# luo-yining/CFDBench

Hardware: AMD Instinct MI355X
Metric: train frames/sec (64x64x2), Auto-FNO cavity (higher is better)
Workload: dtype f32; 1 GPU; BASELINE configs[1]: Auto-FNO train step (fwd+nMSE+bwd+Adam), Fno2d(L=4,hidden=20,modes=12,p=5), 64x64, batch 256/GPU, fp32, random-init weights; act_pieces=3, global_batch=256, parallelism=dp1, graph=False, settle_steps=30

## Files before the change

cfdbench_amd/csrc/cfd_common.h:

```cpp
#pragma once
#include <cfd_intrinsics.h>
#include <hip/hip_runtime.h>

#include "../../include/cfdbench_amd.h"

void cfd_set_error(const char* fmt, ...);

enum { CFD_TUNE_MIX_NWV = 0, CFD_TUNE_WGRAD_WG, CFD_TUNE_FUSED_VARIANT, CFD_TUNE_BLOCK_FUSE, CFD_TUNE_GENERAL_B3, CFD_TUNE_HEAD_BLOCKS, CFD_TUNE_EXACT_FP32, CFD_TUNE_CONV6_GRID, CFD_TUNE_CONV6_WGRAD_MUL, CFD_TUNE_CONVT_MFMA, CFD_TUNE_CONV1_MFMA, CFD_TUNE_SIDE_STREAM, CFD_TUNE_ACT_PIECES, CFD_TUNE_BLOCK_GEN,
    CFD_TUNE_GEMM_TILE, CFD_TUNE_GEMM_SPLITS, CFD_TUNE_BLOCK_WIDE, CFD_TUNE_HEAD_WAVES, CFD_TUNE_STEM_FUSE, CFD_TUNE_MODE_MFMA, CFD_TUNE_MODE_BC, CFD_TUNE_STEM_DFT, CFD_TUNE_GEMM_B3, CFD_TUNE_COUNT };
int cfd_tune_get(int which);

#define CFD_REQUIRE(cond, code, ...)      \
    do {                                  \
        if (!(cond)) {                    \
            cfd_set_error(__VA_ARGS__);   \
            return (code);                \
        }                                 \
    } while (0)

#define CFD_REQUIRE_ALIGNED(ptr, bytes, fn, name) \
    CFD_REQUIRE(((size_t)(ptr) & (size_t)((bytes) - 1)) == 0, CFD_ERR_UNSUPPORTED, "%s: %s must be %d-byte aligned", fn, name, (int)(bytes))

#define CFD_LAUNCH_CHECK(name)                                                        \
    do {                                                                              \
        hipError_t e_ = hipGetLastError();                                            \
        if (e_ != hipSuccess) {                                                       \
            cfd_set_error("%s: HIP launch failed: %s", name, hipGetErrorString(e_));  \
            return CFD_ERR_HIP;                                                       \
        }                                                                             \
    } while (0)

#define CFD_TRY(expr)              \
    do {                           \
        int rc_ = (expr);          \
        if (rc_ != CFD_OK) return rc_; \
    } while (0)

hipStream_t cfd_side_fork(hipStream_t main, int use);
int cfd_side_join(hipStream_t main, hipStream_t side);
bool cfd_prof_active();

struct CfdProfScope {
    hipStream_t st;
    int idx;
    CfdProfScope(const char* name, hipStream_t s, double bytes = 0.0, double flops = 0.0);
    ~CfdProfScope();
};
#define CFD_PROF_CAT2(a, b) a##b
#define CFD_PROF_CAT(a, b) CFD_PROF_CAT2(a, b)
#define CFD_PROF(name, st) CfdProfScope CFD_PROF_CAT(cfd_prof_scope_, __LINE__)(name, st)
#define CFD_PROF_W(name, st, bytes, flops) \
    CfdProfScope CFD_PROF_CAT(cfd_prof_scope_, __LINE__)(name, st, (double)(bytes), (double)(flops))

#define CFD_KB_TMAX 5
struct cfd_plan {
    int H, W, m1, m2;
    int NJ;
    int KX;
    int T;
    int SA;
    int SB;
    int n_fwd, n_inv;
    float* d_fwd;
    float* d_inv;
    void* d_fwd_b3;
    void* d_inv_b3;
    int E;
    float* d_tail;
    void* d_fwd_g;
    void* d_inv_g;
    int NJG, NHG, n_fwd_gv, n_inv_gv;
    float* d_clhw;
    float* d_gx;
    float* d_gy;
    int many;
    float* d_many_fwd;
    float* d_many_inv;
};

struct CfdManyDims {
    int Hk, Hp, Wk, Wq, N1p, K2, R2p, R4;
};
__host__ __device__ static inline CfdManyDims cfd_many_dims(int H, int W, int m1, int m2) {
    CfdManyDims d;
    d.Hk = (H + 3) / 4 * 4;
    d.Hp = (H + 15) / 16 * 16;
    d.Wk = (W + 3) / 4 * 4;
    d.Wq = (W + 15) / 16 * 16;
    d.N1p = (2 * m2 + 15) / 16 * 16;
    d.K2 = (2 * m2 + 3) / 4 * 4;
    d.R2p = (2 * m1 + 15) / 16 * 16;
    d.R4 = (2 * m1 + 3) / 4 * 4;
    return d;
}
int cfd_int_dft_many(const cfd_plan* p, const float* x, float* xh, int nimg, int act_in, void* stream);
int cfd_int_idft_many(const cfd_plan* p, const float* z, const float* addend, const float* aprev, float* out, int nimg, int epi, void* stream);

static inline size_t cfd_align_up(size_t v, size_t a) { return (v + a - 1) / a * a; }

#define CFD_DT_F32 0
#define CFD_DT_BF16 1
template <typename TA>
__device__ __forceinline__ float cfd_ld(const TA* p) { return (float)*p; }
template <typename TA>
__device__ __forceinline__ void cfd_st(TA* p, float v) { *p = (TA)v; }
static inline size_t cfd_dt_size(int dt) { return dt == CFD_DT_BF16 ? 2 : 4; }
__device__ __forceinline__ float4 cfd_ld4(const float* p) { return *reinterpret_cast<const float4*>(p); }
__device__ __forceinline__ float4 cfd_ld4(const __bf16* p) {
    typedef __bf16 bf16x4_ __attribute__((ext_vector_type(4)));
    const bf16x4_ t = *reinterpret_cast<const bf16x4_*>(p);
    return make_float4((float)t[0], (float)t[1], (float)t[2], (float)t[3]);
}

struct __attribute__((packed, aligned(4))) cfd_f4u { float x, y, z, w; };
__device__ __forceinline__ float4 cfd_ld4u(const float* p) {
    const cfd_f4u v = *reinterpret_cast<const cfd_f4u*>(p);
    return make_float4(v.x, v.y, v.z, v.w);
}
__device__ __forceinline__ void cfd_st4u(float* p, float4 v) { *reinterpret_cast<cfd_f4u*>(p) = cfd_f4u{v.x, v.y, v.z, v.w}; }

int cfd_int_spectral_dft(const cfd_plan* p, const void* x, float* xh, int nimg, int act_in, int dt, void* stream);
bool cfd_int_dft_stem_ok(const cfd_plan* p, int B, int in_chan, int P, int C, const void* inputs, const void* mask, const void* a0);
int cfd_int_spectral_dft_stem(const cfd_plan* p, const float* inputs, const float* mask, const float* cp, const float* w, const float* bias,
                              float* a0, float* xh, int B, int P, int C, void* stream);
int cfd_int_spectral_idft(const cfd_plan* p, const float* z, const void* addend, const void* aprev, void* out, int nimg, int epi,
                          int dt, void* stream);
int cfd_int_spectral_idft_grad(const cfd_plan* p, const float* z, const float* addend, const void* aprev, float* out, int nimg,
                               int dt, void* stream);
int cfd_int_chanmix(const void* in, const float* w, const float* bias, void* out, int B, int Ci, int Co, int HW, int act_in,
                    int transpose, int dt, void* stream);
int cfd_int_fno_stem_fwd(const cfd_plan* p, const float* inputs, const float* mask, const float* case_params, const float* w,
                         const float* bias, void* out, int B, int in_chan, int P, int C, int dt, void* stream);
int cfd_int_fno_head_fwd(const void* a, const float* mask, const float* label, const float* w1, const float* b1, const float* w2,
                         const float* b2, float* preds, float* sums, void* ws, int B, int C, int Hd, int Co, int HW, int act_in,
                         int dt, void* stream);

#define CFD_PAD_COORD_GY 128
#define CFD_PAD_COORD_FLOATS 256
int cfd_int_stem_pad(const float* inputs, const float* mask, const float* case_params, const float* w, const float* bias, float* out,
                     float* coords, int B, int in_chan, int P, int C, int H, int W, int pad, void* stream);
int cfd_int_pad_crop(const float* in, float* out, long n, int H, int W, int pad, void* stream);
int cfd_int_pad_embed(const float* in, float* out, long n, int H, int W, int pad, void* stream);

int cfd_int_fno_ingrad(const float* g0, const float* w, float* d_inputs, float* d_case_params, void* ws, size_t ws_bytes, int B, int in_chan,
                       int P, int C, int HW, void* stream);

#define CFD_WIDE_MAX 128
int cfd_int_wide_mix(const cfd_plan* p, const float* xh, const float* w1, const float* w2, float* z, int B, int Cin, int Cout,
                     int conj_t, void* stream);
int cfd_int_wide_wgrad(const cfd_plan* p, const float* xh, const float* gh, float* gw1, float* gw2, int B, int Cin, int Cout,
                       void* stream);
int cfd_int_wide_chanmix(const float* in, const float* w, const float* bias, float* out, int B, int Ci, int Co, int HW, int act_in,
                         int transpose, void* stream, const float* dgelu = nullptr);
size_t cfd_int_wide_chan_wgrad_workspace_bytes(int B, int Ci, int Co, int HW);
int cfd_int_wide_chan_wgrad(const float* g, const float* in, float* gw, float* gb, void* ws, int B, int Ci, int Co, int HW, int act_in,
                            void* stream);
int cfd_int_wide_stem_bwd(const cfd_plan* p, const float* g, const float* inputs, const float* mask, const float* case_params, float* gw,
                          float* gb, void* ws, int B, int in_chan, int P, int C, void* stream);
int cfd_int_wide_head_bwd(const float* a, const float* mask, const float* label, const float* preds, const float* gext, const float* coef,
                          const float* w1, const float* b1, const float* w2, float* ga, float* gw1, float* gb1, float* gw2, float* gb2,
                          void* ws, int B, int C, int Co, int HW, int act_in, void* stream);
int cfd_int_wide_stem_fwd(const cfd_plan* p, const float* inputs, const float* mask, const float* case_params, const float* w,
// ... 298 lines not shown
```

cfdbench_amd/csrc/pointwise.hip:

```cpp
#include "cfd_common.h"
#include "cfd_tail.h"

template <int CP, typename TA>
__global__ __launch_bounds__(256) void k_stem_fwd(const float* __restrict__ inputs, const float* __restrict__ mask,
                                                  const float* __restrict__ cp, const float* __restrict__ gx,
                                                  const float* __restrict__ gy, const float* __restrict__ w,
                                                  const float* __restrict__ bias, TA* __restrict__ out, int B,
                                                  int in_chan, int P, int C, int H, int W) {
    __shared__ float s_w[32 * CP];
    __shared__ float s_b[CP];
    const int F = in_chan + 3 + P;
    {
        constexpr int NV = (32 * CP + 255) / 256;
        float wv[NV];
#pragma unroll
        for (int k = 0; k < NV; ++k) {
            const int i = threadIdx.x + 256 * k, f = i / CP, o = i % CP;
            wv[k] = w[(o < C ? o : C - 1) * F + (f < F ? f : F - 1)];
        }
        float bv = bias[(int)threadIdx.x < C ? threadIdx.x : C - 1];
#pragma unroll
        for (int k = 0; k < NV; ++k) {
            const int i = threadIdx.x + 256 * k, f = i / CP, o = i % CP;
            wv[k] = cfd_opaque_f(wv[k]);
// ... 443 lines not shown
    const size_t ea = sizeof(TA);
    const int vec = (HW % 4 == 0 && ((uintptr_t)in % (4 * ea)) == 0 && ((uintptr_t)out % 16) == 0)   ? 4
                    : (HW % 2 == 0 && ((uintptr_t)in % (2 * ea)) == 0 && ((uintptr_t)out % 8) == 0) ? 2
                                                                                                    : 1;
    CFD_PROF_W(transpose ? "k_chanmix_t" : (act ? "k_chanmix_act" : "k_chanmix"), st, B * HW * ((double)ea * Ci + 4.0 * Co),
               2.0 * B * HW * (double)Ci * Co);
    const bool ap3 = sizeof(TA) == 4 && cfd_act_pieces() == 3;
#define CFD_CB3_P(M_, V_, A_, P_) \
    hipLaunchKernelGGL((k_chanmix_b3<M_, V_, A_, TA, P_>), dim3(blocks), dim3(256), 0, st, in, w, bias, out, B, Ci, Co, HW, transpose)
#define CFD_CB3(M_, V_, A_)                                                                   \
    do {                                                                                      \
        if constexpr (sizeof(TA) == 4) { if (ap3) CFD_CB3_P(M_, V_, A_, 3); else CFD_CB3_P(M_, V_, A_, 2); } \
        else CFD_CB3_P(M_, V_, A_, 2);                                                        \
    } while (0)
#define CFD_CB3_V(M_)                                                      \
    do {                                                                   \
        if (vec == 4) { if (act) CFD_CB3(M_, 4, true); else CFD_CB3(M_, 4, false); } \
        else if (vec == 2) { if (act) CFD_CB3(M_, 2, true); else CFD_CB3(M_, 2, false); } \
        else { if (act) CFD_CB3(M_, 1, true); else CFD_CB3(M_, 1, false); }  \
    } while (0)
    if (Co <= 16) CFD_CB3_V(1);
    else CFD_CB3_V(2);
#undef CFD_CB3_V
#undef CFD_CB3
#undef CFD_CB3_P
    CFD_LAUNCH_CHECK("cfd_chanmix");
    return CFD_OK;
}

template <int CPO, int VEC>
static int launch_chanmix(const float* in, const float* w, const float* bias, float* out, int B, int Ci, int Co, int HW,
                          int act, int transpose, hipStream_t st) {
    const long total = (long)B * (HW / VEC);
    int blocks = (int)((total + 255) / 256);
    if (blocks > 4096) blocks = 4096;
    CFD_PROF_W(transpose ? "k_chanmix_t" : (act ? "k_chanmix_act" : "k_chanmix"), st, 4.0 * B * HW * ((double)Ci + Co),
               2.0 * B * HW * (double)Ci * Co);
    if (act)
        hipLaunchKernelGGL((k_chanmix<CPO, VEC, true>), dim3(blocks), dim3(256), 0, st, in, w, bias, out, B, Ci, Co, HW, transpose);
    else
        hipLaunchKernelGGL((k_chanmix<CPO, VEC, false>), dim3(blocks), dim3(256), 0, st, in, w, bias, out, B, Ci, Co, HW, transpose);
    CFD_LAUNCH_CHECK("cfd_chanmix");
    return CFD_OK;
}

int cfd_int_chanmix(const void* in, const float* w, const float* bias, void* out, int B, int Ci, int Co, int HW, int act_in,
                    int transpose, int dt, void* stream) {
    if (dt == CFD_DT_F32) return cfd_chanmix((const float*)in, w, bias, (float*)out, B, Ci, Co, HW, act_in, transpose, stream);
    CFD_REQUIRE(in && w && out && B >= 0 && Ci >= 1 && Co >= 1 && HW >= 1 && Ci <= 32 && Co <= 32, CFD_ERR_INVALID_ARG, "cfd_chanmix: bad arguments");
    if (B == 0) return CFD_OK;
    hipStream_t st = (hipStream_t)stream;
    if (cfd_tune_get(CFD_TUNE_EXACT_FP32) != 1)
        return launch_chanmix_b3<__bf16>((const __bf16*)in, w, bias, (float*)out, B, Ci, Co, HW, act_in, transpose, st);
    const int VEC = HW % 2 == 0 ? 2 : 1;
    const long total = (long)B * (HW / VEC);
    int blocks = (int)((total + 255) / 256);
    if (blocks > 4096) blocks = 4096;
    CFD_PROF_W(act_in ? "k_chanmix_act" : "k_chanmix", st, B * HW * (2.0 * Ci + 4.0 * Co), 2.0 * B * HW * (double)Ci * Co);
#define CFD_CMB(CPV, VW, A_)                                                                                                  \
    hipLaunchKernelGGL((k_chanmix<CPV, VW, A_, __bf16, float>), dim3(blocks), dim3(256), 0, st, (const __bf16*)in, w, bias, (float*)out, B, \
                       Ci, Co, HW, transpose)
#define CFD_CMB_VA(CPV)                                                    \
    do {                                                                   \
        if (VEC == 2) { if (act_in) CFD_CMB(CPV, 2, true); else CFD_CMB(CPV, 2, false); } \
        else { if (act_in) CFD_CMB(CPV, 1, true); else CFD_CMB(CPV, 1, false); }          \
    } while (0)
    if (Co <= 8) CFD_CMB_VA(8);
    else if (Co <= 16) CFD_CMB_VA(16);
    else if (Co <= 24) CFD_CMB_VA(24);
    else CFD_CMB_VA(32);
#undef CFD_CMB_VA
#undef CFD_CMB
    CFD_LAUNCH_CHECK("cfd_chanmix(bf16 storage)");
    return CFD_OK;
}

extern "C" int cfd_chanmix(const float* in, const float* w, const float* bias, float* out, int B, int Ci, int Co, int HW,
                           int act_in, int transpose, void* stream) {
    CFD_REQUIRE(in && w && out, CFD_ERR_INVALID_ARG, "cfd_chanmix: NULL pointer");
    CFD_REQUIRE(B >= 0 && Ci >= 1 && Co >= 1 && HW >= 1, CFD_ERR_INVALID_ARG, "cfd_chanmix: bad sizes");
    CFD_REQUIRE(Ci <= CFD_WIDE_MAX && Co <= CFD_WIDE_MAX, CFD_ERR_UNSUPPORTED, "cfd_chanmix: Ci=%d Co=%d (max %d) unsupported", Ci, Co,
                CFD_WIDE_MAX);
    if (B == 0) return CFD_OK;
    if (Ci > 32 || Co > 32) return cfd_int_wide_chanmix(in, w, bias, out, B, Ci, Co, HW, act_in, transpose, stream);
    hipStream_t st = (hipStream_t)stream;
    if (cfd_tune_get(CFD_TUNE_EXACT_FP32) != 1)
        return launch_chanmix_b3<float>(in, w, bias, out, B, Ci, Co, HW, act_in, transpose, st);
    const bool v4 = HW % 4 == 0 && ((uintptr_t)in % 16) == 0 && ((uintptr_t)out % 16) == 0;
    const bool v2 = HW % 2 == 0 && ((uintptr_t)in % 8) == 0 && ((uintptr_t)out % 8) == 0;
#define CFD_CM(CPV, VW)                                                                               \
    return (VW == 4 && v4) ? launch_chanmix<CPV, VW>(in, w, bias, out, B, Ci, Co, HW, act_in, transpose, st) \
           : v2            ? launch_chanmix<CPV, 2>(in, w, bias, out, B, Ci, Co, HW, act_in, transpose, st)  \
                           : launch_chanmix<CPV, 1>(in, w, bias, out, B, Ci, Co, HW, act_in, transpose, st)
    if (Co <= 8) CFD_CM(8, 4);
    if (Co <= 16) CFD_CM(16, 4);
    if (Co <= 24) CFD_CM(24, 2);
    CFD_CM(32, 2);
#undef CFD_CM
}

struct StemSrc {
    const float* mask;
    const float* cp;
    const float* gx;
    const float* gy;
    int in_chan, P, W;
};

template <int VEC>
__device__ __forceinline__ void cfd_ld8px(const float* __restrict__ src, int px, int hw, bool ok, float (&v)[8]) {
#pragma unroll
    for (int j = 0; j < 8; ++j) v[j] = 0.f;
    if (!ok) return;
    if constexpr (VEC == 4) {
#pragma unroll
        for (int k = 0; k < 2; ++k)
            if (px + 4 * k < hw) {
                const float4 t = *reinterpret_cast<const float4*>(src + 4 * k);
                v[4 * k] = t.x; v[4 * k + 1] = t.y; v[4 * k + 2] = t.z; v[4 * k + 3] = t.w;
            }
    } else {
#pragma unroll
        for (int k = 0; k < 2; ++k) {
            if (px + 4 * k + 3 < hw) {
                const float4 t = cfd_ld4u(src + 4 * k);
                v[4 * k] = t.x; v[4 * k + 1] = t.y; v[4 * k + 2] = t.z; v[4 * k + 3] = t.w;
            } else {
#pragma unroll
                for (int j = 0; j < 4; ++j)
                    if (px + 4 * k + j < hw) v[4 * k + j] = src[4 * k + j];
            }
        }
    }
}

template <int VEC>
__device__ __forceinline__ void cfd_ld8px(const __bf16* __restrict__ src, int px, int hw, bool ok, float (&v)[8]) {
#pragma unroll
    for (int j = 0; j < 8; ++j) v[j] = 0.f;
    if (!ok) return;
    if constexpr (VEC == 4) {
        if (px + 4 < hw) {
            const bf16x8 t = *reinterpret_cast<const bf16x8*>(src);
#pragma unroll
            for (int j = 0; j < 8; ++j) v[j] = (float)t[j];
        } else if (px < hw) {
#pragma unroll
            for (int j = 0; j < 4; ++j) v[j] = (float)src[j];
        }
    } else {
#pragma unroll
        for (int j = 0; j < 8; ++j)
            if (px + j < hw) v[j] = (float)src[j];
    }
}

template <int MT, int NT, int VEC, bool ACT, bool STEM, typename TIN, int AP>
__global__ __launch_bounds__(256) void k_chan_wgrad(const float* __restrict__ g, const TIN* __restrict__ in,
                                                    StemSrc ss, float* __restrict__ part, int B, int Ci, int Co,
                                                    int HW) {
    __shared__ float s_red[4 * MT * NT * 4 * 64];
    const int lane = threadIdx.x & 63, wave = threadIdx.x >> 6;
    const int q = lane >> 4, n = lane & 15;
    const f32x4 zero = {0.f, 0.f, 0.f, 0.f};
    f32x4 acc[MT][NT];
#pragma unroll
    for (int a = 0; a < MT; ++a)
#pragma unroll
        for (int c = 0; c < NT; ++c) acc[a][c] = zero;
    const int cpb = (HW + 31) / 32;
    const int total = B * cpb;
    const int CiIn = STEM ? ss.in_chan : Ci;
    auto load = [&](int ch, float (&av)[MT][8], float (&bv)[NT][8]) {
        const int b = (int)((unsigned)ch / (unsigned)cpb);
        const int px = (ch - b * cpb) * 32 + 8 * q;
#pragma unroll
        for (int a = 0; a < MT; ++a) {
            const int o = 16 * a + n;
            const float* src = g + ((size_t)b * Co + (o < Co ? o : 0)) * HW + px;
            cfd_ld8px<VEC>(src, px, HW, o < Co, av[a]);
        }
#pragma unroll
        for (int c = 0; c < NT; ++c) {
            const int i = 16 * c + n;
            if (i < CiIn) {
                const TIN* src = in + ((size_t)b * CiIn + i) * HW + px;
                cfd_ld8px<VEC>(src, px, HW, true, bv[c]);
            } else {
                const int f = STEM ? i - ss.in_chan : -1;
                const int row0 = STEM ? px / ss.W : 0, col0 = STEM ? px - row0 * ss.W : 0;
                const bool same_row = STEM && (ss.W % 8 == 0);
                if constexpr (STEM && VEC == 4) {
                    if (same_row && (((uintptr_t)ss.mask | (uintptr_t)ss.gy) % 16) == 0) {
                        const float* p8 = nullptr;
                        const float* p1 = nullptr;
                        float s = 0.f;
                        if (i == Ci) s = 1.f;
                        else if (f == 0) { if (ss.mask) p8 = ss.mask + (size_t)b * HW + px; else s = 1.f; }
                        else if (f == 1) p1 = ss.gx + row0;
                        else if (f == 2) p8 = ss.gy + col0;
                        else if (f < 3 + ss.P) p1 = ss.cp + (size_t)b * ss.P + (f - 3);
                        float4 t0 = make_float4(0.f, 0.f, 0.f, 0.f), t1 = t0;
                        if (p8) {
                            if (px < HW) t0 = *reinterpret_cast<const float4*>(p8);
                            if (px + 4 < HW) t1 = *reinterpret_cast<const float4*>(p8 + 4);
                        } else {
                            if (p1) s = *p1;
                            if (px < HW) t0 = make_float4(s, s, s, s);
                            if (px + 4 < HW) t1 = make_float4(s, s, s, s);
                        }
                        bv[c][0] = t0.x; bv[c][1] = t0.y; bv[c][2] = t0.z; bv[c][3] = t0.w;
                        bv[c][4] = t1.x; bv[c][5] = t1.y; bv[c][6] = t1.z; bv[c][7] = t1.w;
                        continue;
                    }
                }
                float cval = 0.f;
                const float* plane = nullptr;
                const float* tab = nullptr;
                bool by_row = false;
                if (i == Ci) cval = 1.f;
                else if constexpr (STEM) {
                    if (f == 0) { if (ss.mask) plane = ss.mask + (size_t)b * HW + px; else cval = 1.f; }
                    else if (f == 1) { tab = ss.gx; by_row = true; }
                    else if (f == 2) tab = ss.gy;
                    else if (f < 3 + ss.P) cval = ss.cp[(size_t)b * ss.P + (f - 3)];
                }
                if (plane) {
                    if (((uintptr_t)ss.mask % (4 * VEC)) == 0) cfd_ld8px<VEC>(plane, px, HW, true, bv[c]);
                    else cfd_ld8px<1>(plane, px, HW, true, bv[c]);
                } else if (tab) {
                    int row = row0, col = col0;
#pragma unroll
                    for (int j = 0; j < 8; ++j) {
                        bv[c][j] = (px + j < HW) ? tab[by_row ? row : col] : 0.f;
                        if (++col >= ss.W) { col = 0; ++row; }
                    }
                } else {
#pragma unroll
                    for (int j = 0; j < 8; ++j) bv[c][j] = (px + j < HW) ? cval : 0.f;
                }
            }
        }
    };
    const int stride = (int)gridDim.x * 4;
    int ch = (int)blockIdx.x * 4 + wave;
    float av[MT][8], bv[NT][8], avn[MT][8], bvn[NT][8];
    if (ch < total) load(ch, av, bv);
    while (ch < total) {
        const int nx = ch + stride;
        if (nx < total) load(nx, avn, bvn);
        cfd_sched_fence();
        if constexpr (ACT) {
#pragma unroll
            for (int c = 0; c < NT; ++c)
                if (16 * c + n < CiIn) {
#pragma unroll
                    for (int j = 0; j < 8; j += 2) { const cfd_f2 g2 = cfd_gelu2(cfd_f2{bv[c][j], bv[c][j + 1]}); bv[c][j] = g2.x; bv[c][j + 1] = g2.y; }
                }
        }
        {
            CfdAct8<AP> as[MT], bs[NT];
#pragma unroll
            for (int a = 0; a < MT; ++a) as[a] = cfd_act_split8<AP>(av[a]);
#pragma unroll
            for (int c = 0; c < NT; ++c) bs[c] = cfd_act_split8<AP>(bv[c]);
#pragma unroll
            for (int k = 0; k < cfd_nterm_aa(AP); ++k)
#pragma unroll
                for (int a = 0; a < MT; ++a)
#pragma unroll
                    for (int c = 0; c < NT; ++c)
                        acc[a][c] = cfd_mfma16x16x32_bf16(as[a].p[cfd_term_aa_a(AP, k)], bs[c].p[cfd_term_aa_b(AP, k)], acc[a][c]);
        }
        cfd_sched_fence();
#pragma unroll
        for (int a = 0; a < MT; ++a)
#pragma unroll
            for (int j = 0; j < 8; ++j) av[a][j] = avn[a][j];
#pragma unroll
        for (int c = 0; c < NT; ++c)
#pragma unroll
            for (int j = 0; j < 8; ++j) bv[c][j] = bvn[c][j];
        ch = nx;
    }
#pragma unroll
    for (int a = 0; a < MT; ++a)
#pragma unroll
        for (int c = 0; c < NT; ++c)
#pragma unroll
            for (int r = 0; r < 4; ++r) s_red[((wave * MT * NT + a * NT + c) * 4 + r) * 64 + lane] = acc[a][c][r];
    __syncthreads();
    const int NW = Ci + 1;
    float* dst = part + (size_t)blockIdx.x * Co * NW;
    const size_t nb = 1;
    for (int e = threadIdx.x; e < MT * NT * 4 * 64; e += blockDim.x) {
        const int ln = e & 63, r = (e >> 6) & 3, tile = e >> 8;
        const int a = tile / NT, c = tile % NT;
        const int o = 16 * a + 4 * (ln >> 4) + r, i = 16 * c + (ln & 15);
        if (o < Co && i < NW) {
            float s = 0.f;
#pragma unroll
            for (int wv = 0; wv < 4; ++wv) s += s_red[((wv * MT * NT + tile) * 4 + r) * 64 + ln];
            dst[(size_t)(o * NW + i) * nb] = s;
        }
    }
}

__global__ __launch_bounds__(256) void k_wgrad_reduce(const float* __restrict__ part, int nblk, float* __restrict__ gw,
                                                      float* __restrict__ gb, int Co, int Ci) {
    __shared__ float s_scr[64];
    chan_wgrad_reduce_group(blockIdx.x, part, nblk, gw, gb, Co, Ci, s_scr);
}

static int wgrad_blocks(int B, int HW) {
    const long chunks = (long)B * ((HW + 31) / 32);
    long blocks = (chunks + 7) / 8;
    if (blocks > 1024) blocks = 1024;
    const long fill = (chunks + 3) / 4 < 256 ? (chunks + 3) / 4 : 256;
    if (blocks < fill) blocks = fill;
    if (blocks < 1) blocks = 1;
    return (int)blocks;
}

extern "C" size_t cfd_chan_wgrad_workspace_bytes(int B, int Ci, int Co, int HW) {
    if (B <= 0) return 0;
    if (Ci > 32 || Co > 32) return cfd_int_wide_chan_wgrad_workspace_bytes(B, Ci, Co, HW);
    return (size_t)wgrad_blocks(B, HW) * Co * (Ci + 1) * sizeof(float);
}

template <bool STEM, typename TIN = float>
static int launch_wgrad(const float* g, const TIN* in, StemSrc ss, float* gw, float* gb, void* ws, int B, int Ci,
                        int Co, int HW, int act, hipStream_t st, ChanWgradTail* defer = nullptr) {
    const int blocks = wgrad_blocks(B, HW);
    CFD_REQUIRE((long)B * ((HW + 31) / 32) < (1L << 30), CFD_ERR_UNSUPPORTED, "cfd_chan_wgrad: B * ceil(HW / 32) = %ld chunks (max 2^30)",
                (long)B * ((HW + 31) / 32));
    const int MT = (Co + 15) / 16, NT = (Ci + 1 + 15) / 16;
    const int vec = sizeof(TIN) == 2 ? ((HW % 8 == 0 && ((uintptr_t)g % 16) == 0 && ((uintptr_t)in % 16) == 0) ? 4 : 1)
                    : (HW % 4 == 0 && ((uintptr_t)g % 16) == 0 && ((uintptr_t)in % 16) == 0)  ? 4
                    : (HW % 2 == 0 && ((uintptr_t)g % 8) == 0 && ((uintptr_t)in % 8) == 0) ? 2
                                                                                            : 1;
    float* part = (float*)ws;
    const bool ap3 = sizeof(TIN) == 4 && cfd_act_pieces() == 3;
#define CFD_WG_P(M_, N_, V_, A_, P_)                                                                             \
    hipLaunchKernelGGL((k_chan_wgrad<M_, N_, V_, A_, STEM, TIN, P_>), dim3(blocks), dim3(256), 0, st, g, in, ss, part, B, \
                       Ci, Co, HW)
#define CFD_WG(M_, N_, V_, A_)                                                                \
    do {                                                                                      \
        if constexpr (sizeof(TIN) == 4) { if (ap3) CFD_WG_P(M_, N_, V_, A_, 3); else CFD_WG_P(M_, N_, V_, A_, 2); } \
        else CFD_WG_P(M_, N_, V_, A_, 2);                                                     \
    } while (0)
#define CFD_WG_VA(M_, N_)                                                                     \
    do {                                                                                      \
        if (vec == 4) { if (act) CFD_WG(M_, N_, 4, true); else CFD_WG(M_, N_, 4, false); }    \
        else if (vec == 2) { if constexpr (sizeof(TIN) == 4) { if (act) CFD_WG(M_, N_, 2, true); else CFD_WG(M_, N_, 2, false); } } \
        else { if (act) CFD_WG(M_, N_, 1, true); else CFD_WG(M_, N_, 1, false); }             \
    } while (0)
    {
    CFD_PROF_W(STEM ? "k_chan_wgrad_stem" : "k_chan_wgrad", st, (double)B * HW * (4.0 * Co + sizeof(TIN) * (STEM ? 3 : Ci)),
               2.0 * B * HW * (double)Co * (Ci + 1));
    if (MT == 1 && NT == 1) CFD_WG_VA(1, 1);
    else if (MT == 1 && NT == 2) CFD_WG_VA(1, 2);
    else if (MT == 2 && NT == 1) CFD_WG_VA(2, 1);
    else if (MT == 2 && NT == 2) CFD_WG_VA(2, 2);
    else if (MT == 2 && NT == 3) CFD_WG_VA(2, 3);
    else if (MT == 1 && NT == 3) CFD_WG_VA(1, 3);
    else {
        cfd_set_error("cfd_chan_wgrad: Co=%d Ci=%d unsupported tile shape", Co, Ci);
        return CFD_ERR_UNSUPPORTED;
    }
    }
#undef CFD_WG_VA
#undef CFD_WG
#undef CFD_WG_P
    CFD_LAUNCH_CHECK("cfd_chan_wgrad");
    if (defer) {
        *defer = ChanWgradTail{(const float*)part, gw, gb, blocks, Co, Ci};
        return CFD_OK;
    }
    CFD_PROF_W("k_wgrad_reduce", st, 0.0, 0.0);
    hipLaunchKernelGGL(k_wgrad_reduce, dim3((Co * (Ci + 1) + 15) / 16), dim3(256), 0, st, (const float*)part, blocks,
                       gw, gb, Co, Ci);
    CFD_LAUNCH_CHECK("cfd_chan_wgrad(reduce)");
    return CFD_OK;
}

extern "C" int cfd_chan_wgrad(const float* g, const float* in, float* gw, float* gb, void* ws, int B, int Ci, int Co,
                              int HW, int act_in, void* stream) {
    CFD_REQUIRE(g && in && gw && ws, CFD_ERR_INVALID_ARG, "cfd_chan_wgrad: NULL pointer");
    CFD_REQUIRE(B >= 1 && Ci >= 1 && Co >= 1 && HW >= 1, CFD_ERR_INVALID_ARG, "cfd_chan_wgrad: bad sizes");
    CFD_REQUIRE(Ci <= CFD_WIDE_MAX && Co <= CFD_WIDE_MAX, CFD_ERR_UNSUPPORTED, "cfd_chan_wgrad: Ci=%d Co=%d (max %d) unsupported", Ci, Co,
                CFD_WIDE_MAX);
    if (Ci > 32 || Co > 32) return cfd_int_wide_chan_wgrad(g, in, gw, gb, ws, B, Ci, Co, HW, act_in, stream);
    StemSrc ss{};
    return launch_wgrad<false>(g, in, ss, gw, gb, ws, B, Ci, Co, HW, act_in, (hipStream_t)stream);
}

int cfd_int_chan_wgrad(const float* g, const float* in, float* gw, float* gb, void* ws, int B, int Ci, int Co, int HW,
                       int act_in, void* stream, ChanWgradTail* defer) {
    return cfd_int_chan_wgrad_dt(g, in, gw, gb, ws, B, Ci, Co, HW, act_in, CFD_DT_F32, stream, defer);
}

int cfd_int_chan_wgrad_dt(const float* g, const void* in, float* gw, float* gb, void* ws, int B, int Ci, int Co, int HW,
                          int act_in, int dt, void* stream, ChanWgradTail* defer) {
    if (defer) defer->part = nullptr;
    CFD_REQUIRE(g && in && gw && ws, CFD_ERR_INVALID_ARG, "cfd_chan_wgrad: NULL pointer");
    CFD_REQUIRE(B >= 1 && Ci >= 1 && Co >= 1 && HW >= 1, CFD_ERR_INVALID_ARG, "cfd_chan_wgrad: bad sizes");
    CFD_REQUIRE(Ci <= CFD_WIDE_MAX && Co <= CFD_WIDE_MAX, CFD_ERR_UNSUPPORTED, "cfd_chan_wgrad: Ci=%d Co=%d (max %d) unsupported", Ci, Co,
                CFD_WIDE_MAX);
    if (Ci > 32 || Co > 32) {
        CFD_REQUIRE(dt == CFD_DT_F32, CFD_ERR_UNSUPPORTED, "cfd_chan_wgrad: bf16 activation storage needs Ci, Co <= 32 (Ci=%d Co=%d)", Ci, Co);
        return cfd_int_wide_chan_wgrad(g, (const float*)in, gw, gb, ws, B, Ci, Co, HW, act_in, stream);
    }
    StemSrc ss{};
    if (dt == CFD_DT_BF16)
        return launch_wgrad<false, __bf16>(g, (const __bf16*)in, ss, gw, gb, ws, B, Ci, Co, HW, act_in, (hipStream_t)stream, defer);
    return launch_wgrad<false>(g, (const float*)in, ss, gw, gb, ws, B, Ci, Co, HW, act_in, (hipStream_t)stream, defer);
}

extern "C" size_t cfd_fno_stem_bwd_workspace_bytes(const cfd_plan* p, int B, int in_chan, int P, int C) {
    if (!p) return 0;
    return cfd_chan_wgrad_workspace_bytes(B, in_chan + 3 + P, C, p->H * p->W);
}

extern "C" int cfd_fno_stem_bwd(const cfd_plan* p, const float* g, const float* inputs, const float* mask,
                                const float* case_params, float* gw, float* gb, void* ws, int B, int in_chan, int P,
                                int C, void* stream) {
    CFD_REQUIRE(p && g && inputs && gw && gb && ws && (P == 0 || case_params), CFD_ERR_INVALID_ARG, "cfd_fno_stem_bwd: NULL pointer");
    CFD_REQUIRE(in_chan + 3 + P <= 32 && C <= CFD_WIDE_MAX, CFD_ERR_UNSUPPORTED, "cfd_fno_stem_bwd: too many features/channels");
    if (C > 32) return cfd_int_wide_stem_bwd(p, g, inputs, mask, case_params, gw, gb, ws, B, in_chan, P, C, stream);
    StemSrc ss{mask, case_params, p->d_gx, p->d_gy, in_chan, P, p->W};
    return launch_wgrad<true>(g, inputs, ss, gw, gb, ws, B, in_chan + 3 + P, C, p->H * p->W, 0, (hipStream_t)stream);
}

#define CFD_LOSS_BLOCKS 256

__global__ __launch_bounds__(256) void k_loss_part(const float* __restrict__ p, const float* __restrict__ l, size_t n,
                                                   float* __restrict__ part) {
    __shared__ float s_r[3 * 4];
    const size_t stride = (size_t)gridDim.x * blockDim.x;
    size_t i = (size_t)blockIdx.x * blockDim.x + threadIdx.x;
    float a = 0.f, b = 0.f, c = 0.f;
    for (; i + 3 * stride < n; i += 4 * stride) {
        float pv[4], lv[4];
#pragma unroll
        for (int k = 0; k < 4; ++k) { pv[k] = p[i + k * stride]; lv[k] = l[i + k * stride]; }
#pragma unroll
        for (int k = 0; k < 4; ++k) {
            const float d = pv[k] - lv[k];
            a = fmaf(d, d, a);
            b += fabsf(d);
            c = fmaf(lv[k], lv[k], c);
        }
    }
    for (; i < n; i += stride) {
        const float lv = l[i], d = p[i] - lv;
        a = fmaf(d, d, a);
        b += fabsf(d);
        c = fmaf(lv, lv, c);
    }
    a = cfd_wave_sum(a); b = cfd_wave_sum(b); c = cfd_wave_sum(c);
    const int lane = threadIdx.x & 63, wave = threadIdx.x >> 6;
    if (lane == 0) { s_r[wave] = a; s_r[4 + wave] = b; s_r[8 + wave] = c; }
    __syncthreads();
    if (threadIdx.x < 3) {
        const float* s = s_r + 4 * threadIdx.x;
        part[blockIdx.x * 3 + threadIdx.x] = (s[0] + s[1]) + (s[2] + s[3]);
    }
}

__global__ __launch_bounds__(64) void k_loss_final(const float* __restrict__ part, int nblk, float count,
                                                   float* __restrict__ sums) {
    const int lane = threadIdx.x;
    float a = 0.f, b = 0.f, c = 0.f;
    for (int k = lane; k < nblk; k += 64) { a += part[k * 3]; b += part[k * 3 + 1]; c += part[k * 3 + 2]; }
    a = cfd_wave_sum(a); b = cfd_wave_sum(b); c = cfd_wave_sum(c);
    if (lane == 0) { sums[0] = a; sums[1] = b; sums[2] = c; sums[3] = count; }
}

extern "C" size_t cfd_loss_workspace_bytes(size_t n) { (void)n; return CFD_LOSS_BLOCKS * 3 * sizeof(float); }

extern "C" int cfd_masked_loss_sums(const float* preds, const float* labels, float* sums, void* ws, size_t n,
                                    void* stream) {
    CFD_REQUIRE(preds && labels && sums && ws, CFD_ERR_INVALID_ARG, "cfd_masked_loss_sums: NULL pointer");
    CFD_REQUIRE(n >= 1, CFD_ERR_INVALID_ARG, "cfd_masked_loss_sums: empty tensors (mean of nothing)");
    hipStream_t st = (hipStream_t)stream;
    hipLaunchKernelGGL(k_loss_part, dim3(CFD_LOSS_BLOCKS), dim3(256), 0, st, preds, labels, n, (float*)ws);
    CFD_LAUNCH_CHECK("cfd_masked_loss_sums(part)");
    hipLaunchKernelGGL(k_loss_final, dim3(1), dim3(64), 0, st, (const float*)ws, CFD_LOSS_BLOCKS, (float)n, sums);
    CFD_LAUNCH_CHECK("cfd_masked_loss_sums(final)");
    return CFD_OK;
}

__global__ __launch_bounds__(256) void k_loss_sums_bwd(const float* __restrict__ p, const float* __restrict__ l,
                                                       const float* __restrict__ gs, float* __restrict__ gp,
                                                       float* __restrict__ gl, size_t n) {
    const float g0 = gs[0], g1 = gs[1], g2 = gs[2];
    for (size_t i = (size_t)blockIdx.x * blockDim.x + threadIdx.x; i < n; i += (size_t)gridDim.x * blockDim.x) {
        const float lv = l[i], d = p[i] - lv;
        const float sg = d > 0.f ? 1.f : (d < 0.f ? -1.f : 0.f);
        const float g = g0 * 2.f * d + g1 * sg;
        if (gp) gp[i] = g;
        if (gl) gl[i] = g2 * 2.f * lv - g;
    }
}

extern "C" int cfd_loss_sums_bwd(const float* preds, const float* labels, const float* gsums, float* gp, float* gl,
                                 size_t n, void* stream) {
    CFD_REQUIRE(preds && labels && gsums, CFD_ERR_INVALID_ARG, "cfd_loss_sums_bwd: NULL pointer");
    if (n == 0 || (!gp && !gl)) return CFD_OK;
    size_t blocks = (n + 255) / 256;
    if (blocks > 2048) blocks = 2048;
    hipLaunchKernelGGL(k_loss_sums_bwd, dim3((unsigned)blocks), dim3(256), 0, (hipStream_t)stream, preds, labels, gsums,
                       gp, gl, n);
    CFD_LAUNCH_CHECK("cfd_loss_sums_bwd");
    return CFD_OK;
}

__global__ void k_loss_scores(const float* __restrict__ sums, float* __restrict__ scores) {
    if (threadIdx.x == 0 && blockIdx.x == 0) {
        const float n = sums[3];
        const float mse = sums[0] / n;
        scores[0] = mse;
        scores[1] = sqrtf(mse);
// ... 796 lines not shown
```

cfdbench_amd/csrc/tune.cpp:

```cpp
#include <atomic>
#include <cstdio>
#include <cstdlib>
#include <cstring>
#include <mutex>

#include "cfd_common.h"

namespace {
struct Knob {
    int id;
    const char* name;
    const char* env;
    std::atomic<int> value;
};
Knob g_knobs[CFD_TUNE_COUNT] = {
    {CFD_TUNE_MIX_NWV, "mix_nwv", "CFD_MIX_NWV", {-1}},
    {CFD_TUNE_WGRAD_WG, "wgrad_wg", "CFD_WGRAD_WG", {-1}},
    {CFD_TUNE_FUSED_VARIANT, "fused_variant", "CFD_FUSED_VARIANT", {-1}},
    {CFD_TUNE_BLOCK_FUSE, "block_fuse", "CFD_BLOCK_FUSE", {-1}},
    {CFD_TUNE_GENERAL_B3, "general_b3", "CFD_GENERAL_B3", {-1}},
    {CFD_TUNE_HEAD_BLOCKS, "head_blocks", "CFD_HEAD_BLOCKS", {-1}},
    {CFD_TUNE_EXACT_FP32, "exact_fp32", "CFD_EXACT_FP32", {-1}},
    {CFD_TUNE_CONV6_GRID, "conv6_grid", "CFD_CONV6_GRID", {-1}},
    {CFD_TUNE_CONV6_WGRAD_MUL, "conv6_wgrad_mul", "CFD_CONV6_WGRAD_MUL", {-1}},
    {CFD_TUNE_CONVT_MFMA, "convt_mfma", "CFD_CONVT_MFMA", {-1}},
    {CFD_TUNE_CONV1_MFMA, "conv1_mfma", "CFD_CONV1_MFMA", {-1}},
    {CFD_TUNE_SIDE_STREAM, "side_stream", "CFD_SIDE_STREAM", {-1}},
    {CFD_TUNE_ACT_PIECES, "act_pieces", "CFD_ACT_PIECES", {-1}},
    {CFD_TUNE_BLOCK_GEN, "block_gen", "CFD_BLOCK_GEN", {-1}},
    {CFD_TUNE_GEMM_TILE, "gemm_tile", "CFD_GEMM_TILE", {-1}},
    {CFD_TUNE_GEMM_SPLITS, "gemm_splits", "CFD_GEMM_SPLITS", {-1}},
    {CFD_TUNE_BLOCK_WIDE, "block_wide", "CFD_BLOCK_WIDE", {-1}},
    {CFD_TUNE_HEAD_WAVES, "head_waves", "CFD_HEAD_WAVES", {-1}},
    {CFD_TUNE_STEM_FUSE, "stem_fuse", "CFD_STEM_FUSE", {-1}},
    {CFD_TUNE_MODE_MFMA, "mode_mfma", "CFD_MODE_MFMA", {-1}},
    {CFD_TUNE_MODE_BC, "mode_bc", "CFD_MODE_BC", {-1}},
    {CFD_TUNE_STEM_DFT, "stem_dft", "CFD_STEM_DFT", {-1}},
    {CFD_TUNE_GEMM_B3, "gemm_b3", "CFD_GEMM_B3", {-1}},
};
std::once_flag g_once;
void read_env() {
    for (int i = 0; i < CFD_TUNE_COUNT; ++i)
        if (g_knobs[i].id != i) {
            fprintf(stderr, "cfdbench_amd: tune.cpp's knob table is out of step with the CFD_TUNE_* enum at entry %d (%s)\n", i, g_knobs[i].name ? g_knobs[i].name : "?");
            abort();
        }
    for (auto& k : g_knobs)
        if (const char* e = getenv(k.env)) k.value.store(atoi(e), std::memory_order_relaxed);
}
}

int cfd_tune_get(int which) {
    if (which < 0 || which >= CFD_TUNE_COUNT) return -1;
    std::call_once(g_once, read_env);
    return g_knobs[which].value.load(std::memory_order_relaxed);
}

int cfd_act_pieces() { return cfd_tune_get(CFD_TUNE_ACT_PIECES) == 2 ? 2 : 3; }

extern "C" int cfd_tune_set(const char* name, int value) {
    CFD_REQUIRE(name != nullptr, CFD_ERR_INVALID_ARG, "cfd_tune_set: NULL name");
    std::call_once(g_once, read_env);
    for (auto& k : g_knobs)
        if (strcmp(k.name, name) == 0) {
            k.value.store(value, std::memory_order_relaxed);
            return CFD_OK;
        }
    cfd_set_error("cfd_tune_set: unknown knob '%s'", name);
    return CFD_ERR_INVALID_ARG;
}
```

Measured before the change: 211,600 frames/s.

## Add grouped-chunk channel wgrad kernel sharing tail channels across waves

Adds a k_chan_wgrad_grp kernel for 1x1 channel weight gradients with 17-24 channels. It loads the main 16 channels per chunk with unguarded vector loads and splits the tail channels (16+) across lane groups covering G chunks. Lane shuffles then rotate those tail values so each chunk's MFMA sees them, which cuts the padded 32-channel loads the 2x2 tile path needs. It also adds a tunable cap on wgrad block count and factors the partial-sum store into a helper. The grouped path is on by default for hidden=20 (G=4) and adds shuffle overhead plus more complex bounds handling.

```diff
diff --git a/cfdbench_amd/csrc/cfd_common.h b/cfdbench_amd/csrc/cfd_common.h
--- a/cfdbench_amd/csrc/cfd_common.h
+++ b/cfdbench_amd/csrc/cfd_common.h
@@ -7,7 +7,8 @@
 void cfd_set_error(const char* fmt, ...);
 
 enum { CFD_TUNE_MIX_NWV = 0, CFD_TUNE_WGRAD_WG, CFD_TUNE_FUSED_VARIANT, CFD_TUNE_BLOCK_FUSE, CFD_TUNE_GENERAL_B3, CFD_TUNE_HEAD_BLOCKS, CFD_TUNE_EXACT_FP32, CFD_TUNE_CONV6_GRID, CFD_TUNE_CONV6_WGRAD_MUL, CFD_TUNE_CONVT_MFMA, CFD_TUNE_CONV1_MFMA, CFD_TUNE_SIDE_STREAM, CFD_TUNE_ACT_PIECES, CFD_TUNE_BLOCK_GEN,
-    CFD_TUNE_GEMM_TILE, CFD_TUNE_GEMM_SPLITS, CFD_TUNE_BLOCK_WIDE, CFD_TUNE_HEAD_WAVES, CFD_TUNE_STEM_FUSE, CFD_TUNE_MODE_MFMA, CFD_TUNE_MODE_BC, CFD_TUNE_STEM_DFT, CFD_TUNE_GEMM_B3, CFD_TUNE_COUNT };
+    CFD_TUNE_GEMM_TILE, CFD_TUNE_GEMM_SPLITS, CFD_TUNE_BLOCK_WIDE, CFD_TUNE_HEAD_WAVES, CFD_TUNE_STEM_FUSE, CFD_TUNE_MODE_MFMA, CFD_TUNE_MODE_BC, CFD_TUNE_STEM_DFT, CFD_TUNE_GEMM_B3, CFD_TUNE_CHAN_WGRAD_GRP,
+    CFD_TUNE_CHAN_WGRAD_BLOCKS, CFD_TUNE_COUNT };
 int cfd_tune_get(int which);
 
 #define CFD_REQUIRE(cond, code, ...)      \
diff --git a/cfdbench_amd/csrc/pointwise.hip b/cfdbench_amd/csrc/pointwise.hip
--- a/cfdbench_amd/csrc/pointwise.hip
+++ b/cfdbench_amd/csrc/pointwise.hip
@@ -619,6 +619,51 @@
 #pragma unroll
         for (int j = 0; j < 8; ++j)
             if (px + j < hw) v[j] = (float)src[j];
+    }
+}
+
+template <int VEC>
+__device__ __forceinline__ void cfd_ld8px_full(const float* __restrict__ src, float (&v)[8]) {
+#pragma unroll
+    for (int k = 0; k < 2; ++k) {
+        const float4 t = VEC == 4 ? *reinterpret_cast<const float4*>(src + 4 * k) : cfd_ld4u(src + 4 * k);
+        v[4 * k] = t.x; v[4 * k + 1] = t.y; v[4 * k + 2] = t.z; v[4 * k + 3] = t.w;
+    }
+}
+template <int VEC>
+__device__ __forceinline__ void cfd_ld8px_full(const __bf16* __restrict__ src, float (&v)[8]) {
+    if constexpr (VEC == 4) {
+        const bf16x8 t = *reinterpret_cast<const bf16x8*>(src);
+#pragma unroll
+        for (int j = 0; j < 8; ++j) v[j] = (float)t[j];
+    } else {
+#pragma unroll
+        for (int j = 0; j < 8; ++j) v[j] = (float)src[j];
+    }
+}
+
+template <int MT, int NT>
+__device__ __forceinline__ void cfd_wgrad_store_partial(const f32x4 (&acc)[MT][NT], float* s_red, float* __restrict__ part, int Ci, int Co) {
+    const int lane = threadIdx.x & 63, wave = threadIdx.x >> 6;
+#pragma unroll
+    for (int a = 0; a < MT; ++a)
+#pragma unroll
+        for (int c = 0; c < NT; ++c)
+#pragma unroll
+            for (int r = 0; r < 4; ++r) s_red[((wave * MT * NT + a * NT + c) * 4 + r) * 64 + lane] = acc[a][c][r];
+    __syncthreads();
+    const int NW = Ci + 1;
+    float* dst = part + (size_t)blockIdx.x * Co * NW;
+    for (int e = threadIdx.x; e < MT * NT * 4 * 64; e += blockDim.x) {
+        const int ln = e & 63, r = (e >> 6) & 3, tile = e >> 8;
+        const int a = tile / NT, c = tile % NT;
+        const int o = 16 * a + 4 * (ln >> 4) + r, i = 16 * c + (ln & 15);
+        if (o < Co && i < NW) {
+            float s = 0.f;
+#pragma unroll
+            for (int wv = 0; wv < 4; ++wv) s += s_red[((wv * MT * NT + tile) * 4 + r) * 64 + ln];
+            dst[(size_t)(o * NW + i)] = s;
+        }
     }
 }
 
@@ -750,27 +795,126 @@
             for (int j = 0; j < 8; ++j) bv[c][j] = bvn[c][j];
         ch = nx;
     }
-#pragma unroll
-    for (int a = 0; a < MT; ++a)
-#pragma unroll
-        for (int c = 0; c < NT; ++c)
-#pragma unroll
-            for (int r = 0; r < 4; ++r) s_red[((wave * MT * NT + a * NT + c) * 4 + r) * 64 + lane] = acc[a][c][r];
-    __syncthreads();
-    const int NW = Ci + 1;
-    float* dst = part + (size_t)blockIdx.x * Co * NW;
-    const size_t nb = 1;
-    for (int e = threadIdx.x; e < MT * NT * 4 * 64; e += blockDim.x) {
-        const int ln = e & 63, r = (e >> 6) & 3, tile = e >> 8;
-        const int a = tile / NT, c = tile % NT;
-        const int o = 16 * a + 4 * (ln >> 4) + r, i = 16 * c + (ln & 15);
-        if (o < Co && i < NW) {
-            float s = 0.f;
-#pragma unroll
-            for (int wv = 0; wv < 4; ++wv) s += s_red[((wv * MT * NT + tile) * 4 + r) * 64 + ln];
-            dst[(size_t)(o * NW + i) * nb] = s;
-        }
-    }
+    cfd_wgrad_store_partial<MT, NT>(acc, s_red, part, Ci, Co);
+}
+
+template <int G, int VEC, bool ACT, typename TIN, int AP>
+__global__ __launch_bounds__(256, 4) void k_chan_wgrad_grp(const float* __restrict__ g, const TIN* __restrict__ in,
+                                                        float* __restrict__ part, int B, int Ci, int Co, int HW) {
+    static_assert(G == 2 || G == 4, "chunks per group");
+    constexpr int LPC = 16 / G;
+    __shared__ float s_red[4 * 2 * 2 * 4 * 64];
+    const int lane = threadIdx.x & 63, wave = cfd_uniform((int)(threadIdx.x >> 6));
+    const int q = lane >> 4, n = lane & 15;
+    const f32x4 zero = {0.f, 0.f, 0.f, 0.f};
+    f32x4 acc[2][2] = {{zero, zero}, {zero, zero}};
+    const int cpb = (HW + 31) / 32;
+    const int total = B * cpb;
+    const int stride = (int)gridDim.x * 4;
+    const bool ones = n == Ci - 16;
+    const unsigned offa = (unsigned)(n * HW + 8 * q) * 4u, offb = (unsigned)(n * HW + 8 * q) * (unsigned)sizeof(TIN);
+    auto load1 = [&](int ch, float (&av)[8], float (&bv)[8], int& remc) {
+        const int b = (int)((unsigned)ch / (unsigned)cpb);
+        const int pxc = (ch - b * cpb) * 32;
+        remc = HW - pxc;
+        const float* ga_ = reinterpret_cast<const float*>(reinterpret_cast<const char*>(g + ((size_t)b * Co * HW + pxc)) + offa);
+        const TIN* gb_ = reinterpret_cast<const TIN*>(reinterpret_cast<const char*>(in + ((size_t)b * Ci * HW + pxc)) + offb);
+        if (remc >= 32) {
+            cfd_ld8px_full<VEC>(ga_, av);
+            cfd_ld8px_full<VEC>(gb_, bv);
+        } else {
+            cfd_ld8px<VEC>(ga_, pxc + 8 * q, HW, true, av);
+            cfd_ld8px<VEC>(gb_, pxc + 8 * q, HW, true, bv);
+        }
+    };
+    auto loadg = [&](int ch, float (&av)[8], float (&bv)[8]) {
+        const int nn = cfd_opaque(n), cc = 16 + (nn & (LPC - 1));
+        const int cs = ch + (nn / LPC) * stride;
+        const bool ok = cs < total;
+        const int b = ok ? (int)((unsigned)cs / (unsigned)cpb) : 0;
+        const int px = ok ? (cs - b * cpb) * 32 + 8 * cfd_opaque(q) : 0;
+        cfd_ld8px<VEC>(g + (((size_t)b * Co + (cc < Co ? cc : 0)) * HW + px), px, HW, ok && cc < Co, av);
+        cfd_ld8px<VEC>(in + (((size_t)b * Ci + (cc < Ci ? cc : 0)) * HW + px), px, HW, ok && cc < Ci, bv);
+    };
+    auto gelu8 = [](float (&v)[8]) {
+#pragma unroll
+        for (int j = 0; j < 8; j += 2) { const cfd_f2 g2 = cfd_gelu2(cfd_f2{v[j], v[j + 1]}); v[j] = g2.x; v[j + 1] = g2.y; }
+    };
+    CfdAct8<AP> gas, gbs;
+    auto rotate = [&](CfdAct8<AP>& s, int mask) {
+#pragma unroll
+        for (int p = 0; p < AP; ++p) {
+            const cfd_u32x4 w = __builtin_bit_cast(cfd_u32x4, s.p[p]);
+            cfd_u32x4 r;
+#pragma unroll
+            for (int j = 0; j < 4; ++j) {
+                const unsigned u = w[j];
+                r[j] = __builtin_bit_cast(unsigned, cfd_shfl_xor(__builtin_bit_cast(float, u), mask));
+            }
+            s.p[p] = __builtin_bit_cast(bf16x8, r);
+        }
+    };
+    auto step = [&](int k, float (&av)[8], float (&bv)[8], int remc) {
+        const int rem = remc >= 32 ? 8 : remc - 8 * q;
+        if constexpr (ACT) gelu8(bv);
+        CfdAct8<AP> as[2], bs[2];
+        as[0] = cfd_act_split8<AP>(av);
+        bs[0] = cfd_act_split8<AP>(bv);
+        if (k > 0) {
+            rotate(gas, (k ^ (k - 1)) * LPC);
+            rotate(gbs, (k ^ (k - 1)) * LPC);
+        }
+        as[1] = gas;
+#pragma unroll
+        for (int p = 0; p < AP; ++p) {
+            const cfd_u32x4 w = __builtin_bit_cast(cfd_u32x4, gbs.p[p]);
+            cfd_u32x4 r;
+#pragma unroll
+            for (int j = 0; j < 4; ++j) {
+                const unsigned u = w[j];
+                const unsigned one = p == 0 ? (rem > 2 * j ? 0x3f80u : 0u) | (rem > 2 * j + 1 ? 0x3f800000u : 0u) : 0u;
+                r[j] = ones ? one : u;
+            }
+            bs[1].p[p] = __builtin_bit_cast(bf16x8, r);
+        }
+#pragma unroll
+        for (int t = 0; t < cfd_nterm_aa(AP); ++t)
+#pragma unroll
+            for (int a = 0; a < 2; ++a)
+#pragma unroll
+                for (int c = 0; c < 2; ++c)
+                    acc[a][c] = cfd_mfma16x16x32_bf16(as[a].p[cfd_term_aa_a(AP, t)], bs[c].p[cfd_term_aa_b(AP, t)], acc[a][c]);
+    };
+    float a0[8], b0[8], a1[8], b1[8], ga[8], gb[8];
+    int r0 = 0, r1 = 0;
+    int ch = (int)blockIdx.x * 4 + wave;
+    if (ch < total) {
+        load1(ch, a0, b0, r0);
+        loadg(ch, ga, gb);
+    }
+    while (ch < total) {
+        if constexpr (ACT) gelu8(gb);
+        gas = cfd_act_split8<AP>(ga);
+        gbs = cfd_act_split8<AP>(gb);
+#pragma unroll
+        for (int k = 0; k < G; k += 2) {
+            int cur = ch + k * stride;
+            if (cur >= total) break;
+            if (cur + stride < total) load1(cur + stride, a1, b1, r1);
+            cfd_sched_fence();
+            step(k, a0, b0, r0);
+            cfd_sched_fence();
+            cur += stride;
+            if (cur >= total) break;
+            if (cur + stride < total) load1(cur + stride, a0, b0, r0);
+            cfd_sched_fence();
+            step(k + 1, a1, b1, r1);
+            cfd_sched_fence();
+        }
+        loadg(ch + G * stride, ga, gb);
+        ch += G * stride;
+    }
+    cfd_wgrad_store_partial<2, 2>(acc, s_red, part, Ci, Co);
 }
 
 __global__ __launch_bounds__(256) void k_wgrad_reduce(const float* __restrict__ part, int nblk, float* __restrict__ gw,
@@ -779,7 +923,7 @@
     chan_wgrad_reduce_group(blockIdx.x, part, nblk, gw, gb, Co, Ci, s_scr);
 }
 
-static int wgrad_blocks(int B, int HW) {
+static int wgrad_blocks_uncapped(int B, int HW) {
     const long chunks = (long)B * ((HW + 31) / 32);
     long blocks = (chunks + 7) / 8;
     if (blocks > 1024) blocks = 1024;
@@ -789,10 +933,16 @@
     return (int)blocks;
 }
 
+static int wgrad_blocks(int B, int HW) {
+    const int blocks = wgrad_blocks_uncapped(B, HW);
+    const int cap = cfd_tune_get(CFD_TUNE_CHAN_WGRAD_BLOCKS);
+    return (cap > 0 && blocks > cap) ? cap : blocks;
+}
+
 extern "C" size_t cfd_chan_wgrad_workspace_bytes(int B, int Ci, int Co, int HW) {
     if (B <= 0) return 0;
     if (Ci > 32 || Co > 32) return cfd_int_wide_chan_wgrad_workspace_bytes(B, Ci, Co, HW);
-    return (size_t)wgrad_blocks(B, HW) * Co * (Ci + 1) * sizeof(float);
+    return (size_t)wgrad_blocks_uncapped(B, HW) * Co * (Ci + 1) * sizeof(float);
 }
 
 template <bool STEM, typename TIN = float>
@@ -822,10 +972,28 @@
         else if (vec == 2) { if constexpr (sizeof(TIN) == 4) { if (act) CFD_WG(M_, N_, 2, true); else CFD_WG(M_, N_, 2, false); } } \
         else { if (act) CFD_WG(M_, N_, 1, true); else CFD_WG(M_, N_, 1, false); }             \
     } while (0)
+    const int grp = (STEM || MT != 2 || NT != 2 || Ci < 17 || Co < 17 || Ci > 24 || Co > 24 || HW >= (1 << 24) || cfd_tune_get(CFD_TUNE_CHAN_WGRAD_GRP) == 0) ? 0
+                    : (Ci <= 20 && Co <= 20)                                                                                              ? 4
+                                                                                                                                          : 2;
+#define CFD_WGG_P(G_, V_, A_, P_) \
+    hipLaunchKernelGGL((k_chan_wgrad_grp<G_, V_, A_, TIN, P_>), dim3(blocks), dim3(256), 0, st, g, in, part, B, Ci, Co, HW)
+#define CFD_WGG(G_, V_, A_)                                                                \
+    do {                                                                                   \
+        if constexpr (sizeof(TIN) == 4) { if (ap3) CFD_WGG_P(G_, V_, A_, 3); else CFD_WGG_P(G_, V_, A_, 2); } \
+        else CFD_WGG_P(G_, V_, A_, 2);                                                     \
+    } while (0)
+#define CFD_WGG_VA(G_)                                                                     \
+    do {                                                                                   \
+        if (vec == 4) { if (act) CFD_WGG(G_, 4, true); else CFD_WGG(G_, 4, false); }       \
+        else if (vec == 2) { if constexpr (sizeof(TIN) == 4) { if (act) CFD_WGG(G_, 2, true); else CFD_WGG(G_, 2, false); } } \
+        else { if (act) CFD_WGG(G_, 1, true); else CFD_WGG(G_, 1, false); }                \
+    } while (0)
     {
-    CFD_PROF_W(STEM ? "k_chan_wgrad_stem" : "k_chan_wgrad", st, (double)B * HW * (4.0 * Co + sizeof(TIN) * (STEM ? 3 : Ci)),
+    CFD_PROF_W(STEM ? "k_chan_wgrad_stem" : grp ? "k_chan_wgrad_grp" : "k_chan_wgrad", st, (double)B * HW * (4.0 * Co + sizeof(TIN) * (STEM ? 3 : Ci)),
                2.0 * B * HW * (double)Co * (Ci + 1));
-    if (MT == 1 && NT == 1) CFD_WG_VA(1, 1);
+    if (grp == 4) { if constexpr (!STEM) CFD_WGG_VA(4); }
+    else if (grp == 2) { if constexpr (!STEM) CFD_WGG_VA(2); }
+    else if (MT == 1 && NT == 1) CFD_WG_VA(1, 1);
     else if (MT == 1 && NT == 2) CFD_WG_VA(1, 2);
     else if (MT == 2 && NT == 1) CFD_WG_VA(2, 1);
     else if (MT == 2 && NT == 2) CFD_WG_VA(2, 2);
@@ -836,6 +1004,9 @@
         return CFD_ERR_UNSUPPORTED;
     }
     }
+#undef CFD_WGG_VA
+#undef CFD_WGG
+#undef CFD_WGG_P
 #undef CFD_WG_VA
 #undef CFD_WG
 #undef CFD_WG_P
diff --git a/cfdbench_amd/csrc/tune.cpp b/cfdbench_amd/csrc/tune.cpp
--- a/cfdbench_amd/csrc/tune.cpp
+++ b/cfdbench_amd/csrc/tune.cpp
@@ -37,6 +37,8 @@
     {CFD_TUNE_MODE_BC, "mode_bc", "CFD_MODE_BC", {-1}},
     {CFD_TUNE_STEM_DFT, "stem_dft", "CFD_STEM_DFT", {-1}},
     {CFD_TUNE_GEMM_B3, "gemm_b3", "CFD_GEMM_B3", {-1}},
+    {CFD_TUNE_CHAN_WGRAD_GRP, "chan_wgrad_grp", "CFD_CHAN_WGRAD_GRP", {-1}},
+    {CFD_TUNE_CHAN_WGRAD_BLOCKS, "chan_wgrad_blocks", "CFD_CHAN_WGRAD_BLOCKS", {-1}},
 };
 std::once_flag g_once;
 void read_env() {
```

Measured after the change: 215,400 frames/s (median of 6 runs). +1.8%, better.
